# weibozhao/flink-ml

Hardware: AMD Instinct MI355X
Metric: samples/sec (whole node), LogisticRegression 10M×1K dense at 1/2/4/8 MI355X (higher is better)
Workload: dtype bf16; 1 GPU; model=LogisticRegression (SGD, binary logistic loss), global_batch=100000, parallelism=dp1, rows=10000000, dim=1000, per_gpu_batch=100000, world_size_observed=1, hipgraph=True, collective=none, round=one fused kernel

## Files before the change

flink_ml_amd/ops/csrc/glm.hip:

```cpp
#include "common.h"
#include "xgmi.h"
#include "glm_core.h"

extern "C" void fmlx_glm_sparse_set_trace(void* trace);

namespace {


struct GlmTail {
  int mode;
  int max_iter;
  int det;
  int flat_lds;
  int nbatch;
  int* cnt;
  void* acc;
  void* stage1;
  void* feedback;
  double tol, lr, reg, en;
  xgmi::Ctx x;
  int red_off;
  int acc_reps;
  long acc_ld;
  int ticket2;
// ... 187 lines not shown
    }
    stop = !(e < tl.max_iter && L / W > (A)tl.tol);
    const A lr = (A)tl.lr, reg = (A)tl.reg, en = (A)tl.en;
    const A* wp = cw + (long)((e - 1) & 1) * d;
    for (long c = tid; c < d; c += nt) {
      A v[ACC_MAX_REPS];
#pragma unroll
      for (int q = 0; q < ACC_MAX_REPS; ++q) v[q] = q < R ? ld_agent(prev + q * ald + c) : (A)0;
      const A w0 = wp[c];
      A g = (A)0;
#pragma unroll
      for (int q = 0; q < ACC_MAX_REPS; ++q) g += v[q];
      wl[c] = sgd_apply<A>(w0, g, W, lr, reg, en);
      if (lead && fb) fb[c] = g;
    }
    if (lead && fb && tid == 0) {
      fb[d] = W;
      fb[d + 1] = L;
    }
  }
  A* nxt = ring + (long)((e + 1) % 3) * slot;
  for (long i = (long)blockIdx.x * nt + tid; i < slot; i += (long)gridDim.x * nt) nxt[i] = (A)0;
  __syncthreads();
  if (lead) {
    A* wc = cw + (long)(e & 1) * d;
    for (long c = tid; c < d; c += nt) {
      wc[c] = wl[c];
      coef[c] = wl[c];
    }
    if (tid == 0) {
      state[tl.parity ? ST_ROUND : ST_ROUND_ALT] = e + 1;
      if (e > 0) state[ST_EXECUTED] += 1;
      if (stop) state[ST_DONE] = 1;
    }
  }
  return stop;
}

constexpr int WFLAG_IDX = 120;
template <typename A>
__device__ bool defer_prologue_xgmi(const GlmTail& tl, A* coef, int* state, int e, int d, A* wl) {
  const int nt = blockDim.x, tid = threadIdx.x;
  const int R = tl.acc_reps > 1 ? tl.acc_reps : 1;
  const long ald = tl.acc_ld;
  const long slot = (long)ACC_MAX_REPS * ald;
  const long stride = d + 2;
  A* ring = (A*)tl.acc;
  A* cw = (A*)tl.cw;
  A* fb = (A*)tl.feedback;
  int* wflag = tl.cnt + WFLAG_IDX;
  __shared__ int s_stop;
  const bool lead = blockIdx.x == 0;
  if (e == 0) {
    for (long c = tid; c < d; c += nt) wl[c] = coef[c];
    if (tid == 0) s_stop = 0;
  } else if (lead) {
    extern __shared__ __align__(16) unsigned char smem_x[];
    A* xr = reinterpret_cast<A*>(smem_x + tl.xb_off);
    const A* prev = ring + (long)((e + 2) % 3) * slot;
    for (long c = tid; c < stride; c += nt) {
      A v[ACC_MAX_REPS];
#pragma unroll
      for (int q = 0; q < ACC_MAX_REPS; ++q) v[q] = q < R ? ld_agent(prev + q * ald + c) : (A)0;
      A g = (A)0;
#pragma unroll
      for (int q = 0; q < ACC_MAX_REPS; ++q) g += v[q];
      xr[c] = g;
    }
    __syncthreads();
    glm_xgmi_exchange<A>(tl.x, xr, stride);
    const A W = xr[d], L = xr[d + 1];
    const bool stop = !(e < tl.max_iter && L / W > (A)tl.tol);
    const A lr = (A)tl.lr, reg = (A)tl.reg, en = (A)tl.en;
    const A* wp = cw + (long)((e - 1) & 1) * d;
    A* wc = cw + (long)(e & 1) * d;
    for (long c = tid; c < d; c += nt) {
      const A w = sgd_apply<A>(wp[c], xr[c], W, lr, reg, en);
      wl[c] = w;
      st_agent(wc + c, w);
      coef[c] = w;
      if (fb) fb[c] = xr[c];
    }
    if (tid == 0) {
      if (fb) {
        fb[d] = W;
        fb[d + 1] = L;
      }
      s_stop = stop;
    }
    asm volatile("s_waitcnt vmcnt(0)" ::: "memory");
    __syncthreads();
    if (tid == 0) st_agent(wflag, (e << 1) | (stop ? 1 : 0));
  } else {
    if (tid == 0) {
      int v = 0;
      long it = 0;
      for (;;) {
        v = ld_agent(wflag);
        if ((v >> 1) == e) break;
        if (++it > 4 * tl.x.spin_limit || ((it & 1023) == 0 && xgmi::ld_sys(tl.x.err) != 0)) {
          xgmi::st_sys(tl.x.err, 1);
          v = (e << 1) | 1;
          break;
        }
        __builtin_amdgcn_s_sleep(2);
      }
      s_stop = v & 1;
    }
    __syncthreads();
    __builtin_amdgcn_fence(__ATOMIC_ACQUIRE, "wavefront");
    if (!s_stop) {
      const A* wc = cw + (long)(e & 1) * d;
      for (long c = tid; c < d; c += nt) wl[c] = ld_agent(wc + c);
    }
  }
  __syncthreads();
  const bool stop = s_stop != 0;
  A* nxt = ring + (long)((e + 1) % 3) * slot;
  for (long i = (long)blockIdx.x * nt + tid; i < slot; i += (long)gridDim.x * nt) nxt[i] = (A)0;
  if (lead && tid == 0) {
    state[tl.parity ? ST_ROUND : ST_ROUND_ALT] = e + 1;
    if (e > 0) state[ST_EXECUTED] += 1;
    if (stop) state[ST_DONE] = 1;
  }
  if (lead && e == 0)
    for (long c = tid; c < d; c += nt) cw[c] = wl[c];
  return stop;
}

template <int L>
__device__ __forceinline__ float seg_sum_dpp(float v) {
  v += dpp_mov<0xB1>(v);
  v += dpp_mov<0x4E>(v);
  v += dpp_mov<0x141>(v);
  if constexpr (L == 16) v += dpp_mov<0x140>(v);
  return v;
}

template <typename T, int EPC, int CPL, int U>
constexpr int glm_min_waves() {
  return sizeof(T) <= 4 && ((U == 1 && CPL * EPC * (int)sizeof(T) <= 32) || (U == 2 && CPL * EPC * (int)sizeof(T) <= 16))
             ? 4
             : 1;
}

__device__ __forceinline__ void dma16_nt(const void* g, unsigned lds) {
  unsigned keep;
  asm volatile("s_mov_b32 %0, m0\n\ts_mov_b32 m0, %2\n\ts_nop 0\n\tglobal_load_lds_dwordx4 %1, off nt\n\ts_mov_b32 m0, %0"
               : "=&s"(keep)
               : "v"(g), "s"(lds)
               : "memory");
}

template <typename T, int EPC, int CPL, int U, int WPB, bool NT, int DEPTH = 0>
__global__ __launch_bounds__(WPB * 64, (glm_min_waves<T, EPC, CPL, U>())) void glm_round_kernel(
    const T* X, long ld, const typename AccOf<T>::type* y,
    const typename AccOf<T>::type* wt, typename AccOf<T>::type* coef,
    long n, int d, long B, int loss, int* state, typename AccOf<T>::type* partials, GlmTail tl) {
  typedef typename AccOf<T>::type A;
  const long long t_start = tl.trace ? (long long)__builtin_amdgcn_s_memrealtime() : 0;
  int e;
  if (tl.defer) {
    if (state[ST_DONE]) return;
    e = state[tl.parity ? ST_ROUND_ALT : ST_ROUND];
  } else if (!round_running(state, e)) return;
  long start = 0, end = 0;
  if (n > 0 && B > 0) {
    const unsigned P = tl.nbatch > 0 ? (unsigned)tl.nbatch : (unsigned)((n + B - 1) / B);
    start = (long)((unsigned)e % P) * B;
    end = start + B < n ? start + B : n;
  }

  const int lane = threadIdx.x & 63;
  const int wave = __builtin_amdgcn_readfirstlane(threadIdx.x >> 6);
  const int nch = d / EPC;
  const long W = (long)gridDim.x * WPB;
  const long gw = (long)blockIdx.x * WPB + wave;

  constexpr bool kPacked = sizeof(T) == 2 && EPC % 2 == 0;
  typedef float f2_t __attribute__((ext_vector_type(2)));
  constexpr int EP = kPacked ? EPC / 2 : 1;
  A w[CPL][EPC];
  A acc[CPL][EPC];
  f2_t w2[CPL][EP], acc2[CPL][EP];
#pragma unroll
  for (int k = 0; k < CPL; ++k) {
#pragma unroll
    for (int i = 0; i < EPC; ++i) acc[k][i] = (A)0;
#pragma unroll
    for (int i = 0; i < EP; ++i) acc2[k][i] = f2_t{0.f, 0.f};
  }
  extern __shared__ __align__(16) unsigned char smem_w[];
  A* wdef = reinterpret_cast<A*>(smem_w + tl.wl_off);
  typedef __attribute__((address_space(3))) A lds_acc_t;
  const lds_acc_t* wlds = (const lds_acc_t*)(smem_w + tl.wl_off);
  auto load_w = [&]() {
    if (tl.defer) {
#pragma unroll
      for (int k = 0; k < CPL; ++k) {
        const int c = lane + 64 * k;
        if constexpr (kPacked) {
#pragma unroll
          for (int i = 0; i < EP; ++i)
            w2[k][i] = c < nch ? f2_t{(float)wlds[c * EPC + 2 * i], (float)wlds[c * EPC + 2 * i + 1]} : f2_t{0.f, 0.f};
        } else {
#pragma unroll
          for (int i = 0; i < EPC; ++i) w[k][i] = c < nch ? wlds[c * EPC + i] : (A)0;
        }
      }
      return;
    }
#pragma unroll
    for (int k = 0; k < CPL; ++k) {
      const int c = lane + 64 * k;
      if constexpr (kPacked) {
#pragma unroll
        for (int i = 0; i < EP; ++i)
          w2[k][i] = c < nch ? f2_t{(float)coef[c * EPC + 2 * i], (float)coef[c * EPC + 2 * i + 1]} : f2_t{0.f, 0.f};
      } else {
#pragma unroll
        for (int i = 0; i < EPC; ++i) w[k][i] = c < nch ? coef[c * EPC + i] : (A)0;
      }
    }
  };
  A wsum = 0, lsum = 0;

  Chunk<T, EPC> xa[U][CPL], xb[U][CPL];
  A ya[U], wa[U], yb[U], wb[U];
  bool va[U], vb[U];
  const bool has_wt = wt != nullptr;
  const A* wsrc = has_wt ? wt : y;
  const long r_first = start + gw;
  A ylab = (A)0, wlab = (A)1;
  auto load_labels = [&](long j0) {
    long rr = r_first + (j0 + lane) * W;
    rr = rr < end ? rr : (end > 0 ? end - 1 : 0);
    ylab = y[rr];
    wlab = wsrc[rr];
  };
  auto lane_val = [&](A v, int l) -> A {
    if constexpr (sizeof(A) == 4) {
      return __int_as_float(__builtin_amdgcn_readlane(__float_as_int(v), l));
    } else {
      const long long b = __double_as_longlong(v);
      const int lo = __builtin_amdgcn_readlane((int)(b & 0xffffffffLL), l);
      const int hi = __builtin_amdgcn_readlane((int)(b >> 32), l);
      return __longlong_as_double(((long long)hi << 32) | (unsigned int)lo);
    }
  };
  auto load_rows = [&](long r0, long j0, long rsafe, Chunk<T, EPC> (&dst)[U][CPL], A (&yy)[U], A (&ww)[U],
                       bool (&vv)[U]) {
    if ((j0 & 63) == 0 && j0 > 0) load_labels(j0);
#pragma unroll
    for (int u = 0; u < U; ++u) {
      const long ru0 = r0 + u * W;
      const bool ok = ru0 < end;
      const long ru = ok ? ru0 : rsafe;
      vv[u] = ok;
      const T* row = X + ru * ld;
#pragma unroll
      for (int k = 0; k < CPL; ++k) {
        const int c = lane + 64 * k;
        if constexpr (NT) load_chunk_nt<T, EPC>(row + (c < nch ? c : nch - 1) * EPC, dst[u][k]);
        else load_chunk<T, EPC>(row + (c < nch ? c : nch - 1) * EPC, dst[u][k]);
      }
    }
#pragma unroll
    for (int u = 0; u < U; ++u) {
      yy[u] = lane_val(ylab, (int)((j0 + u) & 63));
      ww[u] = lane_val(wlab, (int)((j0 + u) & 63));
    }
  };
  auto process = [&](Chunk<T, EPC> (&x)[U][CPL], A (&yy)[U], A (&ww)[U], bool (&vv)[U]) {
    if constexpr (kPacked) {
      f2_t xf[U][CPL][EP];
      A dot[U];
#pragma unroll
      for (int u = 0; u < U; ++u) {
        f2_t s2[2] = {{0.f, 0.f}, {0.f, 0.f}};
#pragma unroll
        for (int k = 0; k < CPL; ++k) {
          const uint32_t* q = reinterpret_cast<const uint32_t*>(x[u][k].v);
#pragma unroll
          for (int i = 0; i < EP; ++i) {
            xf[u][k][i] = f2_t{__uint_as_float(q[i] << 16), __uint_as_float(q[i] & 0xffff0000u)};
            s2[i & 1] = __builtin_elementwise_fma(xf[u][k][i], w2[k][i], s2[i & 1]);
          }
        }
        const f2_t st = s2[0] + s2[1];
        dot[u] = st.x + st.y;
      }
#pragma unroll
      for (int u = 0; u < U; ++u) dot[u] = wave_sum_dpp(dot[u]);
#pragma unroll
      for (int u = 0; u < U; ++u) {
        A l, m;
        const A wu = has_wt ? ww[u] : (A)1;
        loss_and_mult(loss, dot[u], yy[u], wu, l, m);
        if (!vv[u]) { l = (A)0; m = (A)0; }
        wsum += vv[u] ? wu : (A)0;
        lsum += l;
        const f2_t m2 = {m, m};
#pragma unroll
        for (int k = 0; k < CPL; ++k)
#pragma unroll
          for (int i = 0; i < EP; ++i) acc2[k][i] = __builtin_elementwise_fma(m2, xf[u][k][i], acc2[k][i]);
      }
    } else {
      A dot[U];
#pragma unroll
      for (int u = 0; u < U; ++u) {
        A s = 0;
#pragma unroll
        for (int k = 0; k < CPL; ++k)
#pragma unroll
          for (int i = 0; i < EPC; ++i) s += (A)Ld<T>::f(x[u][k].v[i]) * w[k][i];
        dot[u] = s;
      }
#pragma unroll
      for (int u = 0; u < U; ++u) dot[u] = wave_sum_dpp(dot[u]);
#pragma unroll
      for (int u = 0; u < U; ++u) {
        A l, m;
        const A wu = has_wt ? ww[u] : (A)1;
        loss_and_mult(loss, dot[u], yy[u], wu, l, m);
        if (!vv[u]) { l = (A)0; m = (A)0; }
        wsum += vv[u] ? wu : (A)0;
        lsum += l;
#pragma unroll
        for (int k = 0; k < CPL; ++k)
#pragma unroll
          for (int i = 0; i < EPC; ++i) acc[k][i] += m * (A)Ld<T>::f(x[u][k].v[i]);
      }
    }
  };
  if constexpr (DEPTH > 0) {
    static_assert(sizeof(T) == 2 && EPC == 8 && CPL == 2, "LDS-DMA ring: bf16 rows of 65-128 chunks");
    extern __shared__ __align__(16) unsigned char smem_r[];
    typedef unsigned int u32x4_t __attribute__((ext_vector_type(4)));
    typedef __attribute__((address_space(3))) u32x4_t lds_u4_t;
    unsigned char* ring_w = smem_r + tl.ring_off + (long)wave * (DEPTH * U * 2048);
    const unsigned ring_a = __builtin_amdgcn_readfirstlane((unsigned)(size_t)ring_w);
    const long nrw = r_first < end ? (end - r_first + W - 1) / W : 0;
    const long nst = (nrw + U - 1) / U;
    const int c1 = lane + 64 < nch ? lane + 64 : nch - 1;
    auto issue = [&](long t) {
      const unsigned base = ring_a + (unsigned)((t % DEPTH) * U) * 2048u;
#pragma unroll
      for (int u = 0; u < U; ++u) {
        long ru = r_first + (t * U + u) * W;
        ru = ru < end ? ru : r_first;
        const T* row = X + ru * ld;
        dma16_nt(row + lane * EPC, base + u * 2048u);
        dma16_nt(row + c1 * EPC, base + u * 2048u + 1024u);
      }
    };
    auto read = [&](long t, Chunk<T, EPC> (&x)[U][CPL], A (&yy)[U], A (&ww)[U], bool (&vv)[U]) {
      const long j0 = t * U;
      if ((j0 & 63) == 0 && j0 > 0) load_labels(j0);
      const unsigned char* sl = ring_w + (t % DEPTH) * U * 2048;
#pragma unroll
      for (int u = 0; u < U; ++u) {
#pragma unroll
        for (int k = 0; k < CPL; ++k) {
          const u32x4_t v = *(const lds_u4_t*)(sl + u * 2048 + k * 1024 + lane * 16);
          __builtin_memcpy(x[u][k].v, &v, 16);
        }
        vv[u] = j0 + u < nrw;
        yy[u] = lane_val(ylab, (int)((j0 + u) & 63));
        ww[u] = lane_val(wlab, (int)((j0 + u) & 63));
      }
    };
    if (nst > 0) {
      load_labels(0);
#pragma unroll
      for (int t = 0; t < DEPTH - 1; ++t)
        if (t < nst) issue(t);
    }
    if (tl.defer && (tl.mode == TAIL_XGMI ? defer_prologue_xgmi<A>(tl, coef, state, e, d, wdef)
                                          : defer_prologue<A>(tl, coef, state, e, d, wdef))) {
      asm volatile("s_waitcnt vmcnt(0)" ::: "memory");
      return;
    }
    if (nst > 0) {
      load_w();
      for (long t = 0; t < nst; ++t) {
        if (t + DEPTH - 1 < nst) {
          issue(t + DEPTH - 1);
          asm volatile("s_waitcnt vmcnt(%0)" ::"n"(2 * U * (DEPTH - 1)) : "memory");
        } else {
          asm volatile("s_waitcnt vmcnt(0)" ::: "memory");
        }
        read(t, xa, ya, wa, va);
        process(xa, ya, wa, va);
      }
    }
    __syncthreads();
  } else {
  const long step = (long)U * W;
  long r = start + gw;
  const long nst = r < end ? ((end - r + W - 1) / W + U - 1) / U : 0;
  if (nst > 0) {
    load_labels(0);
    load_rows(r, 0, r, xa, ya, wa, va);
    load_rows(r + step, U, r, xb, yb, wb, vb);
  }
  if (tl.defer && (tl.mode == TAIL_XGMI ? defer_prologue_xgmi<A>(tl, coef, state, e, d, wdef)
                                        : defer_prologue<A>(tl, coef, state, e, d, wdef)))
    return;
  if (nst > 0) {
    load_w();
    __builtin_amdgcn_s_waitcnt(0x0F70);
    long t = 0;
    for (; t + 2 <= nst; t += 2) {
      process(xa, ya, wa, va);
      asm volatile("" ::: "memory");
      __builtin_amdgcn_sched_barrier(0);
      load_rows(r + 2 * step, (t + 2) * U, r, xa, ya, wa, va);
      asm volatile("" ::: "memory");
      __builtin_amdgcn_sched_barrier(0);
      process(xb, yb, wb, vb);
      asm volatile("" ::: "memory");
      __builtin_amdgcn_sched_barrier(0);
      load_rows(r + 3 * step, (t + 3) * U, r, xb, yb, wb, vb);
      asm volatile("" ::: "memory");
      __builtin_amdgcn_sched_barrier(0);
      r += 2 * step;
    }
    if (t < nst) process(xa, ya, wa, va);
  }
  }

  if (tl.trace) {
    __syncthreads();
    if (threadIdx.x == 0) {
      long long* tr = tl.trace + (long)blockIdx.x * 4;
      tr[0] = t_start;
      tr[1] = (long long)__builtin_amdgcn_s_memrealtime();
      unsigned hw;
      asm volatile("s_getreg_b32 %0, hwreg(HW_REG_HW_ID)" : "=s"(hw));
      unsigned xcc;
      asm volatile("s_getreg_b32 %0, hwreg(HW_REG_XCC_ID)" : "=s"(xcc));
      tr[3] = ((long long)xcc << 32) | hw;
    }
  }
  if constexpr (kPacked) {
#pragma unroll
    for (int k = 0; k < CPL; ++k)
#pragma unroll
      for (int i = 0; i < EP; ++i) {
        acc[k][2 * i] = acc2[k][i].x;
        acc[k][2 * i + 1] = acc2[k][i].y;
      }
  }

  extern __shared__ __align__(16) unsigned char smem_raw[];
  A* buf = reinterpret_cast<A*>(smem_raw);
  const bool flat = tl.mode != TAIL_PARTIALS && !tl.det && tl.flat_lds;
  A* lw = buf + (flat ? WPB : WPB / 2) * (long)d;
  int* sflag = reinterpret_cast<int*>(lw + WPB * 2);
  if (lane == 0) { lw[wave * 2] = wsum; lw[wave * 2 + 1] = lsum; }
  if (flat) {
    A* mine = buf + (long)wave * d;
#pragma unroll
    for (int k = 0; k < CPL; ++k) {
      const int c = lane + 64 * k;
      if (c < nch)
#pragma unroll
        for (int i = 0; i < EPC; ++i) mine[c * EPC + i] = acc[k][i];
    }
    __syncthreads();
    const int rep = (int)(blockIdx.x % (tl.acc_reps > 1 ? tl.acc_reps : 1));
    A* gacc = (A*)tl.acc + (long)rep * tl.acc_ld + (tl.defer ? (long)(e % 3) * ACC_MAX_REPS * tl.acc_ld : 0L);
    const long stride = d + 2;
    for (long c = threadIdx.x; c < stride; c += blockDim.x) {
      A v = (A)0;
      if (c < d) {
#pragma unroll
        for (int q = 0; q < WPB; ++q) v += buf[(long)q * d + c];
      } else {
#pragma unroll
        for (int q = 0; q < WPB; ++q) v += lw[q * 2 + (int)(c - d)];
      }
      atomicAdd(gacc + c, v);
    }
    if (tl.trace) {
      asm volatile("s_waitcnt vmcnt(0)" ::: "memory");
      __syncthreads();
      if (threadIdx.x == 0) tl.trace[(long)blockIdx.x * 4 + 2] = (long long)__builtin_amdgcn_s_memrealtime();
    }
    if (tl.defer) return;
    glm_round_tail_atomic<A>(tl, d, coef, state, e, buf, sflag);
    return;
  }
#pragma unroll
  for (int half = WPB / 2; half >= 1; half >>= 1) {
    if (wave >= half && wave < 2 * half) {
      A* dst = buf + (long)(wave - half) * d;
#pragma unroll
      for (int k = 0; k < CPL; ++k) {
        const int c = lane + 64 * k;
        if (c < nch)
#pragma unroll
          for (int i = 0; i < EPC; ++i) dst[c * EPC + i] = acc[k][i];
      }
    }
    __syncthreads();
    if (wave < half) {
      const A* src = buf + (long)wave * d;
#pragma unroll
      for (int k = 0; k < CPL; ++k) {
        const int c = lane + 64 * k;
        if (c < nch)
#pragma unroll
          for (int i = 0; i < EPC; ++i) acc[k][i] += src[c * EPC + i];
      }
    }
    __syncthreads();
  }
  if (tl.mode != TAIL_PARTIALS && !tl.det) {
    if (wave == 0) {
#pragma unroll
      for (int k = 0; k < CPL; ++k) {
        const int c = lane + 64 * k;
        if (c < nch)
#pragma unroll
          for (int i = 0; i < EPC; ++i) buf[c * EPC + i] = acc[k][i];
      }
      if (lane == 0) {
        A ws = 0, ls = 0;
        for (int q = 0; q < WPB; ++q) { ws += lw[q * 2]; ls += lw[q * 2 + 1]; }
        buf[d] = ws;
        buf[d + 1] = ls;
      }
    }
    __syncthreads();
    A* gacc = (A*)tl.acc + (long)(blockIdx.x % (tl.acc_reps > 1 ? tl.acc_reps : 1)) * tl.acc_ld;
    for (long c = threadIdx.x; c < d + 2; c += blockDim.x) atomicAdd(gacc + c, buf[c]);
    glm_round_tail_atomic<A>(tl, d, coef, state, e, buf, sflag);
    return;
  }
  if (wave == 0) {
    A* out = partials + (long)blockIdx.x * (d + 2);
    const bool wt1 = tl.mode != TAIL_PARTIALS;
#pragma unroll
    for (int k = 0; k < CPL; ++k) {
      const int c = lane + 64 * k;
      if (c < nch)
#pragma unroll
        for (int i = 0; i < EPC; ++i) {
          if (wt1) st_agent(out + c * EPC + i, acc[k][i]);
          else out[c * EPC + i] = acc[k][i];
        }
    }
    if (lane == 0) {
      A ws = 0, ls = 0;
      for (int q = 0; q < WPB; ++q) { ws += lw[q * 2]; ls += lw[q * 2 + 1]; }
      if (wt1) {
        st_agent(out + d, ws);
        st_agent(out + d + 1, ls);
      } else {
        out[d] = ws;
        out[d + 1] = ls;
      }
    }
  }
  if (tl.mode == TAIL_PARTIALS) return;
  glm_round_tail_det<A>(tl, partials, d, coef, state, e, buf, sflag);
}

constexpr int RED_G = 32;

template <typename A>
__global__ __launch_bounds__(256) void glm_reduce_stage1_kernel(const A* __restrict__ partials, int nparts, int d,
                                                                A* __restrict__ stage1, const int* __restrict__ state) {
  int e;
  if (!round_running(state, e)) return;
  const long stride = d + 2;
  const int c = blockIdx.x * 256 + threadIdx.x;
  if (c >= stride) return;
  const int p0 = blockIdx.y * RED_G;
  A v[RED_G];
#pragma unroll
  for (int q = 0; q < RED_G; ++q) v[q] = (p0 + q < nparts) ? partials[(long)(p0 + q) * stride + c] : (A)0;
  A s = 0;
#pragma unroll
  for (int q = 0; q < RED_G; ++q) s += v[q];
  stage1[(long)blockIdx.y * stride + c] = s;
}

template <typename A>
__device__ __forceinline__ A sum_groups(const A* __restrict__ stage1, int ngroups, long stride, long c) {
  A v[16];
#pragma unroll
  for (int q = 0; q < 16; ++q) v[q] = q < ngroups ? stage1[(long)q * stride + c] : (A)0;
  A s = 0;
#pragma unroll
  for (int q = 0; q < 16; ++q) s += v[q];
  return s;
}


template <typename A>
__global__ __launch_bounds__(256) void glm_reduce_update_kernel(
    const A* __restrict__ stage1, int ngroups, int d, A* __restrict__ coef, A* __restrict__ feedback,
    int* __restrict__ state, int max_iter, A tol, A lr, A reg, A en) {
  int e;
  const bool run = round_running(state, e);
  if (!run) {
    arrive_and_advance(state, e, false, 0);
    return;
  }
  const long stride = d + 2;
  const int c = blockIdx.x * 256 + threadIdx.x;
  __shared__ A wl[2];
  if (threadIdx.x < 2) wl[threadIdx.x] = sum_groups(stage1, ngroups, stride, d + threadIdx.x);
  const A g = c < d ? sum_groups(stage1, ngroups, stride, c) : (A)0;
  __syncthreads();
  const A W = wl[0];
  const A L = wl[1];
// ... 66 lines not shown
    }
    s = wave_sum(s);
    if (lane == 0) {
      const double dot = (double)s;
      if (mode == 0) {
        const double p = 1.0 - 1.0 / (1.0 + exp(dot));
        pred[r] = dot >= 0 ? 1.0 : 0.0;
        raw[2 * r] = 1.0 - p;
        raw[2 * r + 1] = p;
      } else if (mode == 1) {
        pred[r] = dot >= thr ? 1.0 : 0.0;
        raw[2 * r] = dot;
        raw[2 * r + 1] = -dot;
      } else {
        pred[r] = dot;
      }
    }
  }
}

constexpr int WIDE_WAVES = 8;

template <typename T, int EPC, int CPL, int RU>
__global__ __launch_bounds__(WIDE_WAVES * 64) void glm_round_wide_kernel(
    const T* __restrict__ X, long ld, const typename AccOf<T>::type* __restrict__ y,
    const typename AccOf<T>::type* __restrict__ wt, typename AccOf<T>::type* __restrict__ coef, long n, int d, long B,
    int loss, int* __restrict__ state, GlmTail tl) {
  typedef typename AccOf<T>::type A;
  extern __shared__ __align__(16) unsigned char smem_wide[];
  A* sbuf = reinterpret_cast<A*>(smem_wide);
  int* sflag = reinterpret_cast<int*>(sbuf + d + 2);
  __shared__ A pdot[2][WIDE_WAVES][RU];
  int e;
  if (!round_running(state, e)) return;
  long start = 0, end = 0;
  if (n > 0 && B > 0) {
    const unsigned P = tl.nbatch > 0 ? (unsigned)tl.nbatch : (unsigned)((n + B - 1) / B);
    start = (long)((unsigned)e % P) * B;
    end = start + B < n ? start + B : n;
  }
  const int lane = threadIdx.x & 63;
  const int wave = __builtin_amdgcn_readfirstlane(threadIdx.x >> 6);
  const int nch = d / EPC;
  const int per = (nch + WIDE_WAVES - 1) / WIDE_WAVES;
  const int c0 = wave * per;
  const int c1 = c0 + per < nch ? c0 + per : nch;
  A w[CPL][EPC], acc[CPL][EPC];
#pragma unroll
  for (int k = 0; k < CPL; ++k) {
    const int c = c0 + lane + 64 * k;
#pragma unroll
    for (int i = 0; i < EPC; ++i) {
      w[k][i] = c < c1 ? coef[c * EPC + i] : (A)0;
      acc[k][i] = (A)0;
    }
  }
  const long G = gridDim.x;
  const long r0 = start + blockIdx.x;
  const long nrows = r0 < end ? (end - r0 + G - 1) / G : 0;
  const bool has_wt = wt != nullptr;
  A wsum = 0, lsum = 0;
  Chunk<T, EPC> xa[RU][CPL], xb[RU][CPL];
  auto load = [&](long j, Chunk<T, EPC> (&x)[RU][CPL]) {
#pragma unroll
    for (int u = 0; u < RU; ++u) {
      const long jj = j + u < nrows ? j + u : (nrows > 0 ? nrows - 1 : 0);
      const T* row = X + (r0 + jj * G) * ld;
#pragma unroll
      for (int k = 0; k < CPL; ++k) {
        const int c = c0 + lane + 64 * k;
        load_chunk_nt<T, EPC>(row + (c < c1 ? c : (c0 < c1 ? c0 : 0)) * EPC, x[u][k]);
      }
    }
  };
  auto process = [&](long j, Chunk<T, EPC> (&x)[RU][CPL], int par) {
    A part[RU];
#pragma unroll
    for (int u = 0; u < RU; ++u) {
      A s = 0;
#pragma unroll
      for (int k = 0; k < CPL; ++k)
#pragma unroll
        for (int i = 0; i < EPC; ++i) s += (A)Ld<T>::f(x[u][k].v[i]) * w[k][i];
      part[u] = wave_sum(s);
    }
    if (lane == 0)
#pragma unroll
      for (int u = 0; u < RU; ++u) pdot[par][wave][u] = part[u];
    __syncthreads();
#pragma unroll
    for (int u = 0; u < RU; ++u) {
      A dot = 0;
#pragma unroll
      for (int q = 0; q < WIDE_WAVES; ++q) dot += pdot[par][q][u];
      const bool ok = j + u < nrows;
      const long r = r0 + (j + u) * G;
      A l, m;
      const A wu = ok ? (has_wt ? wt[r] : (A)1) : (A)0;
      loss_and_mult(loss, dot, ok ? y[r] : (A)0, wu, l, m);
      if (!ok) { l = (A)0; m = (A)0; }
      if (wave == 0) {
        wsum += wu;
        lsum += l;
      }
#pragma unroll
      for (int k = 0; k < CPL; ++k)
#pragma unroll
        for (int i = 0; i < EPC; ++i) acc[k][i] += m * (A)Ld<T>::f(x[u][k].v[i]);
    }
  };
  if (nrows > 0) {
    load(0, xa);
    load(RU, xb);
    int par = 0;
    for (long j = 0; j < nrows; j += 2 * RU) {
      process(j, xa, par);
      par ^= 1;
      load(j + 2 * RU, xa);
      if (j + RU < nrows) {
        process(j + RU, xb, par);
        par ^= 1;
        load(j + 3 * RU, xb);
      }
    }
  }
  for (long c = threadIdx.x; c < d + 2; c += blockDim.x) sbuf[c] = (A)0;
  __syncthreads();
#pragma unroll
  for (int k = 0; k < CPL; ++k) {
    const int c = c0 + lane + 64 * k;
    if (c < c1)
#pragma unroll
      for (int i = 0; i < EPC; ++i) sbuf[c * EPC + i] = acc[k][i];
  }
  if (wave == 0 && lane == 0) {
    sbuf[d] = wsum;
    sbuf[d + 1] = lsum;
  }
  __syncthreads();
  const int rep = (int)(blockIdx.x % (tl.acc_reps > 1 ? tl.acc_reps : 1));
  A* gacc = (A*)tl.acc + (long)rep * tl.acc_ld;
  for (long c = threadIdx.x; c < d + 2; c += blockDim.x) atomicAdd(gacc + c, sbuf[c]);
  glm_round_tail_atomic<A>(tl, d, coef, state, e, sbuf, sflag);
}

constexpr int WPB = 8;

static long g_lds_pad = -1;
static int g_nt = -1;
static int g_acc_reps = 4;
static int g_ticket2 = 0;
static long long* g_trace = nullptr;

static int g_dma_depth = 0;

template <typename T, int EPC, int CPL, int U, int DEPTH>
int launch_grad_k(const void* X, long ld, const void* y, const void* wt, void* coef, long n, int d, long B, int loss,
                  int* state, void* partials, int nblocks, GlmTail t2, bool nt, hipStream_t s) {
  typedef typename AccOf<T>::type A;
  const size_t tail = (size_t)(t2.flat_lds ? WPB : WPB / 2) * d * sizeof(A) + WPB * 2 * sizeof(A) + 16;
  const size_t ring = (size_t)WPB * DEPTH * U * 2048;
  size_t shmem = tail > ring ? tail : ring;
  t2.ring_off = 0;
  if (t2.defer) {
    t2.wl_off = (int)((shmem + 15) & ~(size_t)15);
    shmem = (size_t)t2.wl_off + (size_t)d * sizeof(A);
    if (t2.mode == TAIL_XGMI) {
      t2.xb_off = (int)((shmem + 15) & ~(size_t)15);
      shmem = (size_t)t2.xb_off + (size_t)(d + 2) * sizeof(A);
    }
  }
  if (g_lds_pad >= 0) {
    shmem += (size_t)g_lds_pad;
  } else {
    const long per_cu = (nblocks + NUM_CU - 1) / NUM_CU;
    if (per_cu <= 3) {
      const size_t want = (size_t)(LDS_PER_CU / (per_cu + 1) + 1024);
      if (shmem < want) shmem = want;
    }
  }
  if (shmem > (size_t)LDS_PER_CU) return -8;
  if constexpr (EPC * sizeof(T) == 16 && sizeof(T) == 2) {
    if (nt) {
      hipLaunchKernelGGL((glm_round_kernel<T, EPC, CPL, U, WPB, true, DEPTH>), dim3(nblocks), dim3(WPB * 64), shmem, s,
                         (const T*)X, ld, (const A*)y, (const A*)wt, (A*)coef, n, d, B, loss, state, (A*)partials, t2);
      return (int)hipGetLastError();
    }
  }
  if constexpr (DEPTH == 0) {
    hipLaunchKernelGGL((glm_round_kernel<T, EPC, CPL, U, WPB, false>), dim3(nblocks), dim3(WPB * 64), shmem, s,
                       (const T*)X, ld, (const A*)y, (const A*)wt, (A*)coef, n, d, B, loss, state, (A*)partials, t2);
    return (int)hipGetLastError();
  }
  return -9;
}

template <typename T, int EPC, int CPL, int U>
int launch_grad_u(const void* X, long ld, const void* y, const void* wt, void* coef, long n, int d, long B, int loss,
                  int* state, void* partials, int nblocks, const GlmTail& tl, int flags, hipStream_t s) {
  typedef typename AccOf<T>::type A;
  GlmTail t2 = tl;
  t2.nbatch = (n > 0 && B > 0) ? (int)((n + B - 1) / B) : 0;
  t2.flat_lds = tl.mode != TAIL_PARTIALS && !tl.det && (size_t)WPB * d * sizeof(A) <= 64 * 1024;
  if (t2.defer && (!t2.flat_lds || (tl.mode != TAIL_UPDATE && tl.mode != TAIL_XGMI) || tl.det || tl.cw == nullptr))
    return -7;
  const bool nt = g_nt >= 0 ? g_nt != 0 : (flags & 1) != 0;
#ifndef FMLX_ISA_PROBE_U
  if constexpr (sizeof(T) == 2 && EPC == 8 && CPL == 2) {
    if (g_dma_depth > 0 && nt) {
      switch (g_dma_depth) {
        case 2: return launch_grad_k<T, EPC, CPL, U, 2>(X, ld, y, wt, coef, n, d, B, loss, state, partials, nblocks, t2, nt, s);
        case 3: return launch_grad_k<T, EPC, CPL, U, 3>(X, ld, y, wt, coef, n, d, B, loss, state, partials, nblocks, t2, nt, s);
        default: return launch_grad_k<T, EPC, CPL, U, 4>(X, ld, y, wt, coef, n, d, B, loss, state, partials, nblocks, t2, nt, s);
      }
    }
  }
#endif
  return launch_grad_k<T, EPC, CPL, U, 0>(X, ld, y, wt, coef, n, d, B, loss, state, partials, nblocks, t2, nt, s);
}

template <typename T, int EPC, int CPL>
int launch_grad(int u, const void* X, long ld, const void* y, const void* wt, void* coef, long n, int d, long B,
                int loss, int* state, void* partials, int nblocks, const GlmTail& tl, int flags, hipStream_t s) {
  constexpr int BYTES = CPL * EPC * (int)sizeof(T);
  if (u <= 0) u = BYTES <= 32 ? 2 : 1;
#ifdef FMLX_ISA_PROBE_U
  return launch_grad_u<T, EPC, CPL, FMLX_ISA_PROBE_U>(X, ld, y, wt, coef, n, d, B, loss, state, partials, nblocks, tl, flags, s);
#endif
  if constexpr (BYTES <= 32) {
    if (u >= 4)
      return launch_grad_u<T, EPC, CPL, 4>(X, ld, y, wt, coef, n, d, B, loss, state, partials, nblocks, tl, flags, s);
  }
  if constexpr (BYTES <= 32) {
    if (u >= 2)
      return launch_grad_u<T, EPC, CPL, 2>(X, ld, y, wt, coef, n, d, B, loss, state, partials, nblocks, tl, flags, s);
  }
  return launch_grad_u<T, EPC, CPL, 1>(X, ld, y, wt, coef, n, d, B, loss, state, partials, nblocks, tl, flags, s);
}

#ifndef FMLX_ISA_PROBE
template <typename T, int EPC>
int launch_grad_cpl(int cpl, int u, const void* X, long ld, const void* y, const void* wt, void* coef, long n, int d,
                    long B, int loss, int* state, void* partials, int nblocks, const GlmTail& tl, int flags,
                    hipStream_t s) {
  switch (cpl) {
    case 1: return launch_grad<T, EPC, 1>(u, X, ld, y, wt, coef, n, d, B, loss, state, partials, nblocks, tl, flags, s);
    case 2: return launch_grad<T, EPC, 2>(u, X, ld, y, wt, coef, n, d, B, loss, state, partials, nblocks, tl, flags, s);
    case 4: return launch_grad<T, EPC, 4>(u, X, ld, y, wt, coef, n, d, B, loss, state, partials, nblocks, tl, flags, s);
    case 8: return launch_grad<T, EPC, 8>(u, X, ld, y, wt, coef, n, d, B, loss, state, partials, nblocks, tl, flags, s);
  }
  return -1;
}

int launch_round(int dtype, int epc, int cpl, int u, const void* X, long ld, const void* y, const void* wt, void* coef,
                 long n, int d, long B, int loss, int* state, void* partials, int nblocks, const GlmTail& tl, int flags,
                 hipStream_t s) {
  if (dtype == DT_BF16) {
    if (epc == 8) return launch_grad_cpl<bf16_t, 8>(cpl, u, X, ld, y, wt, coef, n, d, B, loss, state, partials, nblocks, tl, flags, s);
    if (epc == 4) return launch_grad_cpl<bf16_t, 4>(cpl, u, X, ld, y, wt, coef, n, d, B, loss, state, partials, nblocks, tl, flags, s);
    if (epc == 2) return launch_grad_cpl<bf16_t, 2>(cpl, u, X, ld, y, wt, coef, n, d, B, loss, state, partials, nblocks, tl, flags, s);
    if (epc == 1) return launch_grad_cpl<bf16_t, 1>(cpl, u, X, ld, y, wt, coef, n, d, B, loss, state, partials, nblocks, tl, flags, s);
  } else if (dtype == DT_F32) {
    if (epc == 4) return launch_grad_cpl<float, 4>(cpl, u, X, ld, y, wt, coef, n, d, B, loss, state, partials, nblocks, tl, flags, s);
    if (epc == 2) return launch_grad_cpl<float, 2>(cpl, u, X, ld, y, wt, coef, n, d, B, loss, state, partials, nblocks, tl, flags, s);
    if (epc == 1) return launch_grad_cpl<float, 1>(cpl, u, X, ld, y, wt, coef, n, d, B, loss, state, partials, nblocks, tl, flags, s);
  } else if (dtype == DT_F64) {
    if (epc == 2) return launch_grad_cpl<double, 2>(cpl, u, X, ld, y, wt, coef, n, d, B, loss, state, partials, nblocks, tl, flags, s);
    if (epc == 1) return launch_grad_cpl<double, 1>(cpl, u, X, ld, y, wt, coef, n, d, B, loss, state, partials, nblocks, tl, flags, s);
  }
  return -1;
}

template <typename T, int EPC, int CPL>
int launch_pred(const void* X, long ld, long n, int d, const void* coef, int mode, double thr, double* pred,
                double* raw, hipStream_t s) {
  long waves = n;
  int blocks = (int)((waves + 3) / 4);
  if (blocks > 4096) blocks = 4096;
  if (blocks < 1) blocks = 1;
  hipLaunchKernelGGL((glm_predict_kernel<T, EPC, CPL>), dim3(blocks), dim3(256), 0, s, (const T*)X, ld, n, d,
                     (const typename AccOf<T>::type*)coef, mode, thr, pred, raw);
  return (int)hipGetLastError();
}

template <typename T, int EPC>
int launch_pred_cpl(int cpl, const void* X, long ld, long n, int d, const void* coef, int mode, double thr,
                    double* pred, double* raw, hipStream_t s) {
  switch (cpl) {
    case 1: return launch_pred<T, EPC, 1>(X, ld, n, d, coef, mode, thr, pred, raw, s);
    case 2: return launch_pred<T, EPC, 2>(X, ld, n, d, coef, mode, thr, pred, raw, s);
    case 4: return launch_pred<T, EPC, 4>(X, ld, n, d, coef, mode, thr, pred, raw, s);
    case 8: return launch_pred<T, EPC, 8>(X, ld, n, d, coef, mode, thr, pred, raw, s);
  }
  return -1;
}

#endif
}

#ifdef FMLX_ISA_PROBE
extern "C" int fmlx_glm_isa_probe(int u, const void* X, long ld, const void* y, void* coef, int* state,
                                  const GlmTail* tl) {
  return launch_grad<bf16_t, 8, 2>(u, X, ld, y, nullptr, coef, 1, 1000, 1, 0, state, nullptr, 224, *tl, 1, 0);
}
#else

FMLX_API int fmlx_glm_set_tuning(long lds_pad, int nt) {
  g_lds_pad = lds_pad;
  g_nt = nt;
  return 0;
}

FMLX_API void fmlx_glm_set_trace(void* trace) {
  g_trace = (long long*)trace;
  fmlx_glm_sparse_set_trace(trace);
}

FMLX_API int fmlx_glm_cnt_elems() { return 128; }

FMLX_API int fmlx_glm_set_dma(int depth) {
  if (depth < 0 || depth > 4 || depth == 1) return -1;
  g_dma_depth = depth;
  return 0;
}

FMLX_API int fmlx_glm_set_tail_tuning(int acc_reps, int ticket2) {
  if (acc_reps < 1 || acc_reps > ACC_MAX_REPS) return -1;
  g_acc_reps = acc_reps;
  g_ticket2 = ticket2;
  return 0;
}

FMLX_API long fmlx_glm_acc_elems(int d) { return 3L * ACC_MAX_REPS * (((long)d + 2 + 63) / 64 * 64); }

FMLX_API int fmlx_glm_grad_partials(int dtype, int epc, int cpl, int u, const void* X, long ld, const void* y,
                                    const void* wt, const void* coef, long n, int d, long B, int loss, const int* state,
                                    void* partials, int nblocks, void* stream) {
  GlmTail tl{};
  tl.mode = TAIL_PARTIALS;
  return launch_round(dtype, epc, cpl, u, X, ld, y, wt, const_cast<void*>(coef), n, d, B, loss,
                      const_cast<int*>(state), partials, nblocks, tl, 0, (hipStream_t)stream);
}

FMLX_API int fmlx_glm_round(int dtype, int epc, int cpl, int u, const void* X, long ld, const void* y, const void* wt,
                            void* coef, long n, int d, long B, int loss, int* state, void* partials, int nblocks,
                            int mode, int det, int* cnt, void* acc, void* stage1, void* feedback, int max_iter,
                            double tol, double lr,
                            double reg, double en, void* const* peers, int world, int rank, int* gen, int* err,
                            long spin_limit, int flags, int rounds, int defer, int parity, void* cw,
                            void* stream) {
  if (mode != TAIL_PARTIALS && cnt == nullptr) return -4;
  if (mode != TAIL_PARTIALS && det && (nblocks > TAIL_GROUP * TAIL_MAXG || stage1 == nullptr)) return -4;
  if (mode != TAIL_PARTIALS && !det && (nblocks > TAIL_GROUP * TAIL_TOP || acc == nullptr)) return -4;
  if (mode == TAIL_FEEDBACK && feedback == nullptr) return -5;
  if (mode == TAIL_XGMI && (d + 2 > xgmi::GLM_MAX || peers == nullptr || world > xgmi::MAX_RANKS)) return -6;
  GlmTail tl{};
  tl.mode = mode;
  tl.max_iter = max_iter;
  tl.det = det;
  tl.cnt = cnt;
  tl.acc = acc;
  tl.acc_reps = g_acc_reps;
  tl.acc_ld = ((long)d + 2 + 63) / 64 * 64;
  tl.ticket2 = g_ticket2;
  tl.stage1 = stage1;
  tl.feedback = feedback;
  tl.tol = tol;
  tl.lr = lr;
  tl.reg = reg;
  tl.en = en;
  tl.x = xgmi::Ctx{peers, world, rank, gen, err, spin_limit};
  tl.defer = defer;
  tl.cw = cw;
  tl.trace = g_trace;
  for (int i = 0; i < (rounds > 0 ? rounds : 1); ++i) {
    tl.parity = (parity + i) & 1;
    const int rc = launch_round(dtype, epc, cpl, u, X, ld, y, wt, coef, n, d, B, loss, state, partials, nblocks, tl,
                                flags, (hipStream_t)stream);
    if (rc) return rc;
  }
  return 0;
}

template <typename T, int EPC, int CPL>
static int launch_wide(const void* X, long ld, const void* y, const void* wt, void* coef, long n, int d, long B,
                       int loss, int* state, int nblocks, const GlmTail& tl, hipStream_t s) {
  typedef typename AccOf<T>::type A;
  const size_t lds = (size_t)(d + 2) * sizeof(A) + 16;
  if (lds > (size_t)LDS_PER_CU) return -8;
  hipLaunchKernelGGL((glm_round_wide_kernel<T, EPC, CPL, CPL >= 8 ? 1 : 2>), dim3(nblocks), dim3(WIDE_WAVES * 64), lds,
                     s, (const T*)X,
                     ld, (const A*)y, (const A*)wt, (A*)coef, n, d, B, loss, state, tl);
  return (int)hipGetLastError();
}

template <typename T, int EPC>
static int launch_wide_cpl(int cpl, const void* X, long ld, const void* y, const void* wt, void* coef, long n, int d,
                           long B, int loss, int* state, int nblocks, const GlmTail& tl, hipStream_t s) {
  switch (cpl) {
    case 1: return launch_wide<T, EPC, 1>(X, ld, y, wt, coef, n, d, B, loss, state, nblocks, tl, s);
    case 2: return launch_wide<T, EPC, 2>(X, ld, y, wt, coef, n, d, B, loss, state, nblocks, tl, s);
    case 4: return launch_wide<T, EPC, 4>(X, ld, y, wt, coef, n, d, B, loss, state, nblocks, tl, s);
    case 8: return launch_wide<T, EPC, 8>(X, ld, y, wt, coef, n, d, B, loss, state, nblocks, tl, s);
  }
  return -1;
}

FMLX_API int fmlx_glm_round_wide(int dtype, int epc, int cpl, const void* X, long ld, const void* y, const void* wt,
                                 void* coef, long n, int d, long B, int loss, int* state, int nblocks, int mode,
                                 int* cnt, void* acc, void* feedback, int max_iter, double tol, double lr, double reg,
                                 double en, void* stream) {
  if (mode != TAIL_UPDATE && mode != TAIL_FEEDBACK) return -3;
  if (cnt == nullptr || acc == nullptr || nblocks < 1 || nblocks > TAIL_GROUP * TAIL_TOP) return -4;
  if (mode == TAIL_FEEDBACK && feedback == nullptr) return -5;
  if (d % epc != 0 || (d / epc + WIDE_WAVES - 1) / WIDE_WAVES > 64 * cpl) return -6;
  GlmTail tl{};
  tl.mode = mode;
  tl.max_iter = max_iter;
  tl.cnt = cnt;
  tl.acc = acc;
  tl.acc_reps = g_acc_reps;
  tl.acc_ld = ((long)d + 2 + 63) / 64 * 64;
  tl.ticket2 = g_ticket2;
  tl.feedback = feedback;
  tl.tol = tol;
  tl.lr = lr;
  tl.reg = reg;
  tl.en = en;
  tl.nbatch = (n > 0 && B > 0) ? (int)((n + B - 1) / B) : 0;
  hipStream_t s = (hipStream_t)stream;
  if (dtype == DT_BF16 && epc == 8) return launch_wide_cpl<bf16_t, 8>(cpl, X, ld, y, wt, coef, n, d, B, loss, state, nblocks, tl, s);
  if (dtype == DT_F32 && epc == 4) return launch_wide_cpl<float, 4>(cpl, X, ld, y, wt, coef, n, d, B, loss, state, nblocks, tl, s);
  if (dtype == DT_F64 && epc == 2) return launch_wide_cpl<double, 2>(cpl, X, ld, y, wt, coef, n, d, B, loss, state, nblocks, tl, s);
  return -1;
}

template <typename A>
static int launch_stage1(const void* partials, int nparts, int d, void* stage1, const int* state, hipStream_t s) {
  dim3 grid((d + 2 + 255) / 256, (nparts + RED_G - 1) / RED_G);
  hipLaunchKernelGGL(glm_reduce_stage1_kernel<A>, grid, dim3(256), 0, s, (const A*)partials, nparts, d, (A*)stage1,
                     state);
  return (int)hipGetLastError();
}

FMLX_API int fmlx_glm_reduce_update(int acc_f64, const void* partials, int nparts, int d, void* stage1, void* coef,
                                    void* feedback, int* state, int max_iter, double tol, double lr, double reg,
                                    double en, void* stream) {
  hipStream_t s = (hipStream_t)stream;
  const int ngroups = (nparts + RED_G - 1) / RED_G;
  if (ngroups > 16) return -2;
  int rc = acc_f64 ? launch_stage1<double>(partials, nparts, d, stage1, state, s)
                   : launch_stage1<float>(partials, nparts, d, stage1, state, s);
  if (rc) return rc;
  int blocks = (d + 255) / 256;
  if (acc_f64)
    hipLaunchKernelGGL(glm_reduce_update_kernel<double>, dim3(blocks), dim3(256), 0, s, (const double*)stage1,
                       ngroups, d, (double*)coef, (double*)feedback, state, max_iter, tol, lr, reg, en);
  else
    hipLaunchKernelGGL(glm_reduce_update_kernel<float>, dim3(blocks), dim3(256), 0, s, (const float*)stage1, ngroups,
                       d, (float*)coef, (float*)feedback, state, max_iter, (float)tol, (float)lr, (float)reg,
                       (float)en);
  return (int)hipGetLastError();
}

FMLX_API int fmlx_glm_reduce(int acc_f64, const void* partials, int nparts, int d, void* stage1, void* feedback,
                             const int* state, void* stream) {
  hipStream_t s = (hipStream_t)stream;
  const int ngroups = (nparts + RED_G - 1) / RED_G;
  if (ngroups > 16) return -2;
  int rc = acc_f64 ? launch_stage1<double>(partials, nparts, d, stage1, state, s)
                   : launch_stage1<float>(partials, nparts, d, stage1, state, s);
  if (rc) return rc;
  int blocks = (d + 2 + 255) / 256;
  if (acc_f64)
    hipLaunchKernelGGL(glm_reduce_kernel<double>, dim3(blocks), dim3(256), 0, s, (const double*)stage1, ngroups, d,
                       (double*)feedback, state);
  else
// ... 43 lines not shown
```

flink_ml_amd/ops/glm.py:

```python
from __future__ import annotations

import math
import os
import weakref
from typing import Optional, Tuple

import numpy as np
import torch

from . import native

LOSS_CODES = {"logistic": 0, "hinge": 1, "leastsquare": 2, "ftrl": 3}
MAX_CPL = 8
WPB = 8
GRAD_UNROLL = int(os.environ.get("FMLX_GLM_UNROLL", "0"))
GRAD_BLOCKS = int(os.environ.get("FMLX_GLM_BLOCKS", "0"))


def round_blocks(X) -> int:
    if GRAD_BLOCKS > 0:
        return GRAD_BLOCKS
    lay = pick_layout(X) if X is not None else None
    if lay is not None and GRAD_UNROLL == 0 and lay[0] * lay[1] * X.element_size() == 32:
        return 224
    if lay is not None and (lay[0] * lay[1] * X.element_size() > 32 or X.dtype == torch.float64):
        return 256
    return 512


NT_MIN_BYTES = 256 << 20


def set_tuning(lds_pad: int = -1, nt: int = -1) -> None:
    native.call("fmlx_glm_set_tuning", int(lds_pad), int(nt))


def set_tail_tuning(acc_reps: int = 4, ticket2: bool = False) -> None:
    native.call("fmlx_glm_set_tail_tuning", int(acc_reps), int(bool(ticket2)))


DMA_DEPTH = int(os.environ.get("FMLX_GLM_DMA", "0"))


def set_dma(depth: int) -> None:
    if native.kernels().fmlx_glm_set_dma(int(depth)) != 0:
        raise ValueError("depth must be 0, 2, 3 or 4")


def set_trace(buf: Optional[torch.Tensor]) -> None:
    native.kernels().fmlx_glm_set_trace(native.ptr(buf))


def set_bkt_trace(buf: Optional[torch.Tensor]) -> None:
    if buf is None:
        native.kernels().fmlx_glm_bkt_set_trace(None, 0)
    else:
        assert buf.dtype == torch.int64 and buf.dim() == 2 and buf.shape[1] == 8 and buf.is_contiguous()
        native.kernels().fmlx_glm_bkt_set_trace(native.ptr(buf), int(buf.shape[0]))


def pick_layout(X: torch.Tensor, rounds: bool = True) -> Optional[Tuple[int, int]]:
    if X.dim() != 2:
        return None
    n, d = X.shape
    es = X.element_size()
    ld = X.stride(0)
    if X.stride(1) != 1:
        return None
    base = X.data_ptr()
    for vb in (16, 8, 4, 2):
        epc = vb // es
        if epc < 1:
            continue
        if d % epc == 0 and (ld * es) % vb == 0 and base % vb == 0:
            break
    else:
        return None
    nch = d // epc
    cpl = 1
    while cpl * 64 < nch:
        cpl *= 2
    if cpl > MAX_CPL or (rounds and es == 2 and cpl > 4):
        return None
    return epc, cpl


WIDE_WAVES = 8
WIDE_FUSED = os.environ.get("FMLX_GLM_WIDE_FUSED", "1") == "1"


def pick_wide_layout(X: torch.Tensor) -> Optional[Tuple[int, int]]:
    if X.dim() != 2 or X.stride(1) != 1:
        return None
    es = X.element_size()
    epc = 16 // es
    d = X.shape[1]
    if d % epc or (X.stride(0) * es) % 16 or X.data_ptr() % 16:
        return None
    per = -(-(d // epc) // WIDE_WAVES)
    for cpl in (1, 2, 4, 8):
        if 64 * cpl >= per:
            return epc, cpl
    return None


def wide_blocks_per_cu(X) -> int:
    lay = pick_wide_layout(X)
    return 2 if lay is not None and lay[1] <= 1 else 1


def glm_round_wide(X, y, wt, coef, B: int, loss: int, state, scratch: "RoundScratch", mode: int, feedback,
                   max_iter: int, tol: float, lr: float, reg: float, en: float) -> None:
    epc, cpl = pick_wide_layout(X)
    native.call("fmlx_glm_round_wide", native.dtype_code(X.dtype), epc, cpl, native.ptr(X), X.stride(0), native.ptr(y),
                native.ptr(wt), native.ptr(coef), X.shape[0], X.shape[1], B, loss, native.ptr(state), scratch.nparts,
                mode, native.ptr(scratch.cnt), native.ptr(scratch.acc), native.ptr(feedback), int(max_iter), float(tol),
                float(lr), float(reg), float(en), native.stream_ptr(X.device))


def pad_columns(X: torch.Tensor) -> Optional[torch.Tensor]:
    if X.dim() != 2 or not X.is_cuda:
        return None
    n, d = X.shape
    epc = 16 // X.element_size()
    dp = -(-d // epc) * epc
    nch = dp // epc
    cpl = 1
    while cpl * 64 < nch:
        cpl *= 2
    wide_ok = not DETERMINISTIC and WIDE_FUSED
    if cpl > MAX_CPL and (not wide_ok or -(-nch // WIDE_WAVES) > 64 * 8):
        return None
    need = n * dp * X.element_size()
    free, _ = torch.cuda.mem_get_info(X.device)
    if need > 0.8 * free:
        return None
    Xp = torch.empty((n, dp), dtype=X.dtype, device=X.device)
    Xp[:, d:].zero_()
    Xp[:, :d].copy_(X)
    return Xp if pick_layout(Xp) is not None or wide_ok and pick_wide_layout(Xp) is not None else None


def grad_partials(X, y, wt, coef, B: int, loss: int, state, partials, nblocks: int) -> None:
    epc, cpl = pick_layout(X)
    native.call("fmlx_glm_grad_partials", native.dtype_code(X.dtype), epc, cpl, GRAD_UNROLL, native.ptr(X), X.stride(0),
                native.ptr(y), native.ptr(wt), native.ptr(coef), X.shape[0], X.shape[1], B, loss,
                native.ptr(state), native.ptr(partials), nblocks, native.stream_ptr(X.device))


def stage1_rows(nparts: int) -> int:
    return (nparts + 31) // 32


TAIL_PARTIALS, TAIL_FEEDBACK, TAIL_UPDATE, TAIL_XGMI = 0, 1, 2, 3
TAIL_MAX_BLOCKS = 512
TAIL_MAX_BLOCKS_ATOMIC = 2048
DETERMINISTIC = os.environ.get("FMLX_DETERMINISTIC", "0") == "1"
DEFER = os.environ.get("FMLX_GLM_DEFER", "1") == "1"
DEFER_XGMI = os.environ.get("FMLX_GLM_DEFER_XGMI", "1") == "1"


def defer_supported(d: int, acc: torch.dtype) -> bool:
    es = 8 if acc == torch.float64 else 4
    return DEFER and not DETERMINISTIC and WPB * d * es <= 64 * 1024


def max_round_blocks() -> int:
    return TAIL_MAX_BLOCKS if DETERMINISTIC else TAIL_MAX_BLOCKS_ATOMIC


_dma_applied = False


class RoundScratch:

    def __init__(self, nparts: int, d: int, acc: torch.dtype, device, det: bool = None):
        global _dma_applied
        if not _dma_applied:
            set_dma(DMA_DEPTH)
            _dma_applied = True
        self.nparts = nparts
        self.det = DETERMINISTIC if det is None else bool(det)
        if self.det:
            self.partials = native.zeros((nparts, d + 2), acc, device)
            self.stage1 = native.zeros((stage1_rows(nparts), d + 2), acc, device)
        else:
            self.partials = native.zeros((1, d + 2), acc, device)
            self.stage1 = None
        self.acc = native.zeros(int(native.kernels().fmlx_glm_acc_elems(d)), acc, device)
        self.cnt = native.zeros(int(native.kernels().fmlx_glm_cnt_elems()), torch.int32, device)


def glm_round(X, y, wt, coef, B: int, loss: int, state, scratch: RoundScratch, mode: int, feedback=None,
              max_iter: int = 1, tol: float = 0.0, lr: float = 0.0, reg: float = 0.0, en: float = 0.0,
              xg=None, rounds: int = 1, defer: bool = False, parity: int = 0, cw=None) -> None:
    epc, cpl = pick_layout(X)
    flags = 1 if X.shape[0] * X.stride(0) * X.element_size() > NT_MIN_BYTES else 0
    if xg is not None:
        peers, world, rank, gen, err, spin = xg.kernel_args()
# ... 706 lines not shown
```

Before: 2.610 billion samples/s.

## Add warp-specialized loader wave streaming bf16 rows into LDS ring

Adds a kernel path with one extra loader wave per block. It fills a 4-slot LDS ring using global_load_lds DMA, while the 8 worker waves read rows from LDS and compute the gradient, synchronising through block barriers. The aim is to take global-memory latency off the compute waves and overlap loads with math. This path becomes the default for bf16 with nt set and at most one block per CU. The cost is a barrier every row-group, an idle lane group on the loader wave, and lower occupancy from the larger LDS and the min-waves=1 launch bounds.

Result: faster. 2.701 billion samples/s (median of 6 runs) (+3.5%).

```diff
diff --git a/flink_ml_amd/ops/csrc/glm.hip b/flink_ml_amd/ops/csrc/glm.hip
--- a/flink_ml_amd/ops/csrc/glm.hip
+++ b/flink_ml_amd/ops/csrc/glm.hip
@@ -363,8 +363,11 @@
                : "memory");
 }
 
+constexpr int LOADER = -1;
+constexpr int LOADER_SLOTS = 4;
+constexpr int LOADER_SLOT_BYTES = 16384;
 template <typename T, int EPC, int CPL, int U, int WPB, bool NT, int DEPTH = 0>
-__global__ __launch_bounds__(WPB * 64, (glm_min_waves<T, EPC, CPL, U>())) void glm_round_kernel(
+__global__ __launch_bounds__((WPB + (DEPTH < 0 ? 1 : 0)) * 64, (DEPTH < 0 ? 1 : glm_min_waves<T, EPC, CPL, U>())) void glm_round_kernel(
     const T* X, long ld, const typename AccOf<T>::type* y,
     const typename AccOf<T>::type* wt, typename AccOf<T>::type* coef,
     long n, int d, long B, int loss, int* state, typename AccOf<T>::type* partials, GlmTail tl) {
@@ -607,6 +610,88 @@
       }
     }
     __syncthreads();
+  } else if constexpr (DEPTH < 0) {
+    static_assert(sizeof(T) == 2 && EPC == 8 && CPL == 2 && U == 1, "loader path: bf16 rows of 65-128 chunks, U = 1");
+    constexpr int S = LOADER_SLOTS;
+    constexpr int PIECES = 2 * WPB;
+    static_assert(PIECES * (S - 1) <= 63, "vmcnt counts 63 loads");
+    extern __shared__ __align__(16) unsigned char smem_r[];
+    typedef unsigned int u32x4_t __attribute__((ext_vector_type(4)));
+    typedef __attribute__((address_space(3))) u32x4_t lds_u4_t;
+    unsigned char* ring = smem_r + tl.ring_off;
+    const unsigned ring_a = __builtin_amdgcn_readfirstlane((unsigned)(size_t)ring);
+    const bool loader = wave == WPB;
+    const long rb0 = start + (long)blockIdx.x * WPB;
+    const long nj = rb0 < end ? (end - rb0 + W - 1) / W : 0;
+    const bool dense = ld == (long)d;
+    const int c1 = lane + 64 < nch ? lane + 64 : nch - 1;
+    auto fill = [&](long k) {
+      const unsigned base = ring_a + (unsigned)(k % S) * LOADER_SLOT_BYTES;
+      const long rb = rb0 + k * W;
+      if (dense && rb + WPB <= end) {
+        const T* g = X + rb * ld;
+        const int last = WPB * nch - 1;
+#pragma unroll
+        for (int i = 0; i < PIECES; ++i) {
+          const int c = i * 64 + lane < last ? i * 64 + lane : last;
+          dma16_nt(g + (long)c * EPC, base + i * 1024u);
+        }
+      } else {
+#pragma unroll
+        for (int u = 0; u < WPB; ++u) {
+          const long ru = rb + u < end ? rb + u : rb;
+          const T* row = X + ru * ld;
+          dma16_nt(row + lane * EPC, base + u * 2048u);
+          dma16_nt(row + c1 * EPC, base + u * 2048u + 1024u);
+        }
+      }
+    };
+    if (loader) {
+#pragma unroll
+      for (int k = 0; k < S - 2; ++k)
+        if (k < nj) fill(k);
+    } else if (nj > 0) {
+      load_labels(0);
+    }
+    if (tl.defer && (tl.mode == TAIL_XGMI ? defer_prologue_xgmi<A>(tl, coef, state, e, d, wdef)
+                                          : defer_prologue<A>(tl, coef, state, e, d, wdef))) {
+      asm volatile("s_waitcnt vmcnt(0)" ::: "memory");
+      return;
+    }
+    if (nj > 0) {
+      if (loader) {
+        for (long k = 0; k < nj; ++k) {
+          if (k + S - 2 < nj) {
+            fill(k + S - 2);
+            asm volatile("s_waitcnt vmcnt(%0)" ::"n"(PIECES * (S - 2)) : "memory");
+          } else {
+            asm volatile("s_waitcnt vmcnt(0)" ::: "memory");
+          }
+          __builtin_amdgcn_s_barrier();
+        }
+      } else {
+        load_w();
+        for (long k = 0; k < nj; ++k) {
+          __builtin_amdgcn_s_barrier();
+          asm volatile("" ::: "memory");
+          if ((k & 63) == 0 && k > 0) load_labels(k);
+          const long rb = rb0 + k * W;
+          const unsigned pitch = dense && rb + WPB <= end ? 2u * (unsigned)d : 2048u;
+          const unsigned char* row = ring + (k % S) * LOADER_SLOT_BYTES + wave * pitch;
+          const u32x4_t v0 = *(const lds_u4_t*)(row + lane * 16);
+          const u32x4_t v1 = *(const lds_u4_t*)(row + c1 * 16);
+          asm volatile("s_waitcnt lgkmcnt(0)" ::: "memory");
+          __builtin_amdgcn_sched_barrier(0);
+          __builtin_memcpy(xa[0][0].v, &v0, 16);
+          __builtin_memcpy(xa[0][1].v, &v1, 16);
+          va[0] = rb + wave < end;
+          ya[0] = lane_val(ylab, (int)(k & 63));
+          wa[0] = lane_val(wlab, (int)(k & 63));
+          process(xa, ya, wa, va);
+        }
+      }
+    }
+    __syncthreads();
   } else {
   const long step = (long)U * W;
   long r = start + gw;
@@ -670,13 +755,14 @@
   const bool flat = tl.mode != TAIL_PARTIALS && !tl.det && tl.flat_lds;
   A* lw = buf + (flat ? WPB : WPB / 2) * (long)d;
   int* sflag = reinterpret_cast<int*>(lw + WPB * 2);
-  if (lane == 0) { lw[wave * 2] = wsum; lw[wave * 2 + 1] = lsum; }
+  const bool worker = DEPTH >= 0 || wave < WPB;
+  if (lane == 0 && worker) { lw[wave * 2] = wsum; lw[wave * 2 + 1] = lsum; }
   if (flat) {
     A* mine = buf + (long)wave * d;
 #pragma unroll
     for (int k = 0; k < CPL; ++k) {
       const int c = lane + 64 * k;
-      if (c < nch)
+      if (c < nch && worker)
 #pragma unroll
         for (int i = 0; i < EPC; ++i) mine[c * EPC + i] = acc[k][i];
     }
@@ -1049,14 +1135,16 @@
 static int g_ticket2 = 0;
 static long long* g_trace = nullptr;
 
-static int g_dma_depth = 0;
+static int g_dma_depth = -1;
+static int g_row_path = 0;
 
 template <typename T, int EPC, int CPL, int U, int DEPTH>
 int launch_grad_k(const void* X, long ld, const void* y, const void* wt, void* coef, long n, int d, long B, int loss,
                   int* state, void* partials, int nblocks, GlmTail t2, bool nt, hipStream_t s) {
   typedef typename AccOf<T>::type A;
   const size_t tail = (size_t)(t2.flat_lds ? WPB : WPB / 2) * d * sizeof(A) + WPB * 2 * sizeof(A) + 16;
-  const size_t ring = (size_t)WPB * DEPTH * U * 2048;
+  const size_t ring = DEPTH < 0 ? (size_t)LOADER_SLOTS * LOADER_SLOT_BYTES : (size_t)WPB * DEPTH * U * 2048;
+  constexpr int NW = WPB + (DEPTH < 0 ? 1 : 0);
   size_t shmem = tail > ring ? tail : ring;
   t2.ring_off = 0;
   if (t2.defer) {
@@ -1079,7 +1167,7 @@
   if (shmem > (size_t)LDS_PER_CU) return -8;
   if constexpr (EPC * sizeof(T) == 16 && sizeof(T) == 2) {
     if (nt) {
-      hipLaunchKernelGGL((glm_round_kernel<T, EPC, CPL, U, WPB, true, DEPTH>), dim3(nblocks), dim3(WPB * 64), shmem, s,
+      hipLaunchKernelGGL((glm_round_kernel<T, EPC, CPL, U, WPB, true, DEPTH>), dim3(nblocks), dim3(NW * 64), shmem, s,
                          (const T*)X, ld, (const A*)y, (const A*)wt, (A*)coef, n, d, B, loss, state, (A*)partials, t2);
       return (int)hipGetLastError();
     }
@@ -1104,7 +1192,13 @@
   const bool nt = g_nt >= 0 ? g_nt != 0 : (flags & 1) != 0;
 #ifndef FMLX_ISA_PROBE_U
   if constexpr (sizeof(T) == 2 && EPC == 8 && CPL == 2) {
+    if (g_dma_depth < 0 && nt && nblocks <= NUM_CU) {
+      const int rc = launch_grad_k<T, EPC, CPL, 1, LOADER>(X, ld, y, wt, coef, n, d, B, loss, state, partials, nblocks, t2, nt, s);
+      g_row_path = LOADER;
+      if (rc != -8) return rc;
+    }
     if (g_dma_depth > 0 && nt) {
+      g_row_path = g_dma_depth < 4 ? g_dma_depth : 4;
       switch (g_dma_depth) {
         case 2: return launch_grad_k<T, EPC, CPL, U, 2>(X, ld, y, wt, coef, n, d, B, loss, state, partials, nblocks, t2, nt, s);
         case 3: return launch_grad_k<T, EPC, CPL, U, 3>(X, ld, y, wt, coef, n, d, B, loss, state, partials, nblocks, t2, nt, s);
@@ -1113,6 +1207,7 @@
     }
   }
 #endif
+  g_row_path = 0;
   return launch_grad_k<T, EPC, CPL, U, 0>(X, ld, y, wt, coef, n, d, B, loss, state, partials, nblocks, t2, nt, s);
 }
 
@@ -1216,10 +1311,12 @@
 FMLX_API int fmlx_glm_cnt_elems() { return 128; }
 
 FMLX_API int fmlx_glm_set_dma(int depth) {
-  if (depth < 0 || depth > 4 || depth == 1) return -1;
+  if (depth < -1 || depth > 4 || depth == 1) return -1;
   g_dma_depth = depth;
   return 0;
 }
+
+FMLX_API int fmlx_glm_row_path() { return g_row_path; }
 
 FMLX_API int fmlx_glm_set_tail_tuning(int acc_reps, int ticket2) {
   if (acc_reps < 1 || acc_reps > ACC_MAX_REPS) return -1;
diff --git a/flink_ml_amd/ops/glm.py b/flink_ml_amd/ops/glm.py
--- a/flink_ml_amd/ops/glm.py
+++ b/flink_ml_amd/ops/glm.py
@@ -39,12 +39,16 @@
     native.call("fmlx_glm_set_tail_tuning", int(acc_reps), int(bool(ticket2)))
 
 
-DMA_DEPTH = int(os.environ.get("FMLX_GLM_DMA", "0"))
+DMA_DEPTH = int(os.environ.get("FMLX_GLM_DMA", "-1"))
 
 
 def set_dma(depth: int) -> None:
     if native.kernels().fmlx_glm_set_dma(int(depth)) != 0:
-        raise ValueError("depth must be 0, 2, 3 or 4")
+        raise ValueError("depth must be -1, 0, 2, 3 or 4")
+
+
+def row_path() -> int:
+    return int(native.kernels().fmlx_glm_row_path())
 
 
 def set_trace(buf: Optional[torch.Tensor]) -> None:
```
